# RuoyuFeng/CCEdit

Hardware: AMD Instinct MI355X
Metric: UNet denoising steps/s (TV2V 17x512x768, bf16, CFG-doubled batch) (higher is better)
Workload: dtype bf16; 1 GPU; TV2V depth-midas, 17x512x768, one network evaluation = ControlNet2D + pseudo-3D UNet on B=2 (cfg 7.5 uncond+cond) x T=17 frames, latent 64x96, 77x768 text context; 77.68 TFLOP/step; a 30-step DPMPP2SAncestral clip = 59 such steps + VAE decode; parallelism=single GPU, hint_stem=recomputed every step

## Files before the change

ccedit_amd/csrc/common.h:

```cpp
#pragma once
#include <hip/hip_runtime.h>
#include <stdint.h>

#include "../../include/ccedit_hip.h"

typedef __bf16 bf16;
typedef __attribute__((ext_vector_type(8))) __bf16 bf16x8;
typedef __attribute__((ext_vector_type(4))) __bf16 bf16x4;
typedef __attribute__((ext_vector_type(2))) __bf16 bf16x2;
typedef __attribute__((ext_vector_type(16))) float f32x16;
typedef __attribute__((ext_vector_type(4))) float f32x4;
typedef __attribute__((ext_vector_type(2))) float f32x2;
typedef __attribute__((ext_vector_type(4))) short s16x4;
typedef __attribute__((ext_vector_type(4))) uint32_t u32x4;
typedef __attribute__((ext_vector_type(2))) uint32_t u32x2;

#define GLOBAL_AS __attribute__((address_space(1)))
#define LDS_AS __attribute__((address_space(3)))

__device__ __forceinline__ void glds16(const void* gsrc, void* lds_wave_base) {
    __builtin_amdgcn_global_load_lds((const GLOBAL_AS void*)gsrc, (LDS_AS void*)lds_wave_base, 16, 0, 0);
}

__device__ __forceinline__ float bf2f(bf16 v) { return (float)v; }
__device__ __forceinline__ bf16 f2bf(float v) { return (bf16)v; }

__device__ __forceinline__ float silu_f(float v) { return v * __builtin_amdgcn_rcpf(1.0f + __expf(-v)); }
#ifdef CCEDIT_GELU_AS71_28
__device__ __forceinline__ float gelu_erf_f(float v) {
    const float x = fabsf(v) * 0.70710678118654752440f;
    float p = fmaf(x, 0.0000430638f, 0.0002765672f);
    p = fmaf(x, p, 0.0001520143f);
    p = fmaf(x, p, 0.0092705272f);
    p = fmaf(x, p, 0.0422820123f);
    p = fmaf(x, p, 0.0705230784f);
    p = fmaf(x, p, 1.0f);
    p = p * p;
    p = p * p;
    p = p * p;
    p = p * p;
    const float e = 1.0f - __builtin_amdgcn_rcpf(p);
    return 0.5f * v + 0.5f * fabsf(v) * e;
}
#else
__device__ __forceinline__ float gelu_erf_f(float v) {
    const float vc = __builtin_amdgcn_fmed3f(v, -9.0f, 9.0f);
    const float t = vc * vc;
    float p = fmaf(t, 0.00101426306f, -0.106775724f);
    p = fmaf(t, p, -2.30112134f);
    const float e = __builtin_amdgcn_exp2f(p * vc);
    return v * __builtin_amdgcn_rcpf(1.0f + e);
}
#endif

__device__ __forceinline__ float wave_sum(float v) {
#pragma unroll
    for (int o = 32; o > 0; o >>= 1) v += __shfl_xor(v, o, 64);
    return v;
}

struct CcPolicy {
    int conv_halo = 1;
    int g8 = 1;
    int g8_conv = 1;
    int g8_temporal = 1;
    int g8_split = -1;
    int g8_mfma16 = 1;
    int lin320 = 1;
    int lin320s = 1;
    int lin640 = 1;
    int temp320 = 1;
    int attn_short = 1;
    int attn_text = 1;
    int attn_spatial = 1;
    int attn_pv16 = 1;
    int attn_opt = 1;
    int gn_flat = 1;
    int gn_apply_flat = 1;
    int f32_split = 1;
};
const CcPolicy& cc_policy();

void cc_set_error(const char* fmt, ...);
void cc_note_kernel(const char* fmt, ...);

#define CC_CHECK_ARG(cond, ...)          \
    do {                                 \
        if (!(cond)) {                   \
            cc_set_error(__VA_ARGS__);   \
            return CCEDIT_EINVAL;        \
        }                                \
    } while (0)

#define CC_UNSUPPORTED(cond, ...)        \
    do {                                 \
        if (cond) {                      \
            cc_set_error(__VA_ARGS__);   \
            return CCEDIT_EUNSUPPORTED;  \
        }                                \
    } while (0)

static inline int cc_max_dynamic_lds(const void* fn, int bytes, unsigned long long* done, const char* what) {
    int dev = 0;
    hipError_t e = hipGetDevice(&dev);
    if (e == hipSuccess && dev < 64 && ((*done >> dev) & 1ull)) return CCEDIT_OK;
    if (e == hipSuccess) e = hipFuncSetAttribute(fn, hipFuncAttributeMaxDynamicSharedMemorySize, bytes);
    if (e != hipSuccess) {
        cc_set_error("hipFuncSetAttribute(%s): %s", what, hipGetErrorString(e));
        return (int)e;
    }
    if (dev < 64) *done |= 1ull << dev;
    return CCEDIT_OK;
}

template <class... Arms>
// ... 120 lines not shown
```

ccedit_amd/csrc/convhalo.hip:

```cpp
#include "common.h"
#include "gemm_epilogue.h"
#include <stdlib.h>
#include <type_traits>

namespace {

__device__ __attribute__((aligned(64))) char g_zero_page_h[64];

#ifdef CONV_PROBE
constexpr int kProbeWgs = 8192, kProbeStamps = 8;
__device__ unsigned long long g_conv_probe[kProbeWgs * kProbeStamps];
#define CONV_STAMP(i)                                                                                                     \
    do {                                                                                                                  \
        if (threadIdx.x == 0 && blockIdx.x < kProbeWgs) g_conv_probe[blockIdx.x * kProbeStamps + (i)] = __builtin_amdgcn_s_memrealtime(); \
    } while (0)
#else
#define CONV_STAMP(i) \
    do {              \
    } while (0)
#endif

template <int N>
__device__ __forceinline__ void wait_vmcnt_h() {
    asm volatile("s_waitcnt vmcnt(%0)" ::"n"(N) : "memory");
// ... 126 lines not shown
            __builtin_amdgcn_sched_barrier(0);
#pragma unroll
            for (int i = 0; i < TI; ++i)
                if (i == 0 || !narrow) {
#pragma unroll
                    for (int j = 0; j < TJ; ++j)
                        acc[i][j] = __builtin_amdgcn_mfma_f32_32x32x16_bf16(af[ks & 1][i], bfr[ks & 1][j], acc[i][j], 0, 0, 0);
                }
            __builtin_amdgcn_sched_barrier(0);
        }
    };

    CONV_STAMP(0);
    stageW(0, 0);
    stageH(0, 0);
    wait_vmcnt_h<0>();
    __syncthreads();
    CONV_STAMP(1);
    int kt = 0;
    for (int c = 0; c < nc; ++c) {
        for (int t = 0; t < 9; ++t, ++kt) {
            if (kt + 1 < nk) stageW(kt + 1, (kt + 1) & 1);
            const bool pre = (t == 0) && (c + 1 < nc);
            if (pre) stageH(c + 1, (c + 1) & 1);
            compute(kt & 1, c & 1, t);
            if (pre) wait_vmcnt_h<kHaloIssues - 1>(); else wait_vmcnt_h<0>();
            __syncthreads();
        }
    }

    CONV_STAMP(2);
    const int64_t row_base = ((int64_t)frame * d.Hout + y0) * d.Wout + x0;
    gemm_epilogue<WM, WN, TI, TJ, LDS_MAIN>(
        d, acc, smem, ch0,
        [&](int px) -> int64_t {
            const int tx = px & (TW - 1);
            return x0 + tx < d.Wout ? row_base + (int64_t)(px >> tw_log2) * d.Wout + tx : -1;
        },
        (int64_t)frame, narrow);
    CONV_STAMP(3);
#ifdef CONV_PROBE
    if (threadIdx.x == 0 && blockIdx.x < kProbeWgs) {
        unsigned hw_id;
        asm volatile("s_getreg_b32 %0, hwreg(HW_REG_HW_ID)" : "=s"(hw_id));
        unsigned xcc;
        asm volatile("s_getreg_b32 %0, hwreg(HW_REG_XCC_ID)" : "=s"(xcc));
        g_conv_probe[blockIdx.x * kProbeStamps + 4] = ((unsigned long long)xcc << 32) | hw_id;
        g_conv_probe[blockIdx.x * kProbeStamps + 5] = (unsigned long long)ch0;
    }
#endif
}


constexpr int kHaloBytes4 = 192 * 128;

template <int WM, int WN, int TI, int TJ>
__global__ __launch_bounds__(WM* WN * 64) void conv_halo4_kernel(const CcGemmDesc d, int tw_log2_flags) {
    const int tw_log2 = tw_log2_flags & 0xFF;
    constexpr int NT = WM * WN * 64;
    constexpr int BMC = WM * TI * 32, BNP = WN * TJ * 32;
    static_assert(NT == 256 && BNP == 128 && BMC == 128 && TI == 2, "tile geometry");
    constexpr int NS = 4;
    constexpr int W_SUB = BMC * 64;
    constexpr int LDS_MAIN = NS * W_SUB + 2 * kHaloBytes4;
    extern __shared__ __attribute__((aligned(16))) char smem[];
    char* const sW = smem;
    char* const sH = smem + NS * W_SUB;

    const int tid = threadIdx.x;
    const int lane = tid & 63;
    const int wave = __builtin_amdgcn_readfirstlane(tid >> 6);
    const int wm = wave / WN, wn = wave % WN;
    const int TW = 1 << tw_log2, TH = BNP >> tw_log2, HW_ = TW + 2;
    const int tiles_x = (d.Wout + TW - 1) >> tw_log2, tiles_y = d.Hout / TH;
    const int tpf = tiles_x * tiles_y;

    const int ct_n = (d.N + BMC - 1) / BMC;
    const int64_t pt_n = (int64_t)(d.M / (d.Hout * d.Wout)) * tpf;
    const int64_t pt_per_xcd = (pt_n + 7) / 8;
    const int64_t bid = blockIdx.x;
    const int xcd = (int)(bid & 7);
    const int64_t local = bid >> 3;
    const int Q = d.cgroup > 0 ? d.cgroup : ct_n;
    const int64_t gsz = pt_per_xcd * Q;
    const int cg = (int)(local / gsz);
    const int64_t rr = local - cg * gsz;
    const int qn = min(Q, ct_n - cg * Q);
    const int64_t pl = rr / qn;
    const int64_t pt = xcd * pt_per_xcd + pl;
    if (pt >= pt_n) return;
    const int ch0 = (cg * Q + (int)(rr - pl * qn)) * BMC;
    const int frame = (int)(pt / tpf);
    const int tr = (int)(pt - (int64_t)frame * tpf);
    const int y0 = (tr / tiles_x) * TH, x0 = (tr % tiles_x) << tw_log2;

    const bf16* __restrict__ Ap = (const bf16*)d.A;
    const bf16* __restrict__ Wp = (const bf16*)d.W;
    const bf16* zp = (const bf16*)g_zero_page_h;
    const int nc = d.Cin >> 6, nsub = nc * 18;
    const bool narrow = ((tw_log2_flags >> 8) & 1) && (d.N - ch0 <= WM * 32);

    const int f_hy = (tw_log2 == 3) ? 1 : 0;
    const int p = tid & 7, rsub = tid >> 3;
    int64_t hoff[kHaloIssues];
#pragma unroll
    for (int i = 0; i < kHaloIssues; ++i) {
        const int hrow = i * 32 + rsub;
        const int hy = hrow / HW_, hx = hrow - hy * HW_;
        const int iy = y0 + hy - 1, ix = x0 + hx - 1;
        const bool v = hrow < kHaloRows && (unsigned)iy < (unsigned)d.Hin && (unsigned)ix < (unsigned)d.Win;
        const int gsrc = p ^ (((hx >> 1) + ((hy & 1) << 2) * f_hy) & 7);
        hoff[i] = v ? (((int64_t)frame * d.Hin + iy) * d.Win + ix) * d.lda + gsrc * 8 : -1;
    }
    const int p4 = tid & 3, r4 = tid >> 2;
    const int gsrc_w = p4 ^ ((r4 >> 2) & 3);
    const bf16* const wsrc = Wp + (size_t)(ch0 + r4) * d.Kpad + gsrc_w * 8;
    const size_t wsrc64 = (size_t)64 * d.Kpad;

    auto stageH = [&](int c, int buf) {
#pragma unroll
        for (int i = 0; i < kHaloIssues; ++i) {
            const bf16* src = hoff[i] >= 0 ? Ap + hoff[i] + c * 64 : zp;
            glds16(src, sH + buf * kHaloBytes4 + i * (32 * 128) + wave * 1024);
        }
    };

    const int l31 = lane & 31, hi = lane >> 5;
    const int sw_w = (l31 >> 2) & 3;
    int hb[TJ], pty[TJ], ptx[TJ];
#pragma unroll
    for (int j = 0; j < TJ; ++j) {
        const int px = (wn * TJ + j) * 32 + l31;
        pty[j] = px >> tw_log2;
        ptx[j] = px & (TW - 1);
        hb[j] = pty[j] * HW_ + ptx[j];
    }

    f32x16 acc[TI][TJ];
#pragma unroll
    for (int i = 0; i < TI; ++i)
#pragma unroll
        for (int j = 0; j < TJ; ++j)
#pragma unroll
            for (int r = 0; r < 16; ++r) acc[i][j][r] = 0.f;

    CONV_STAMP(0);
    auto kloop = [&](auto NARROWC) {
        constexpr bool NARROW = decltype(NARROWC)::value;
        constexpr int WI = NARROW ? 1 : 2;
        constexpr int NTI = NARROW ? 1 : TI;
        const char* const fa = sW + ((NARROW ? wm * 32 : wm * TI * 32) + l31) * 64;
        auto stageW = [&](int sidx) {
            const bf16* src = wsrc + sidx * 32;
            char* dst = sW + (sidx & (NS - 1)) * W_SUB + wave * 1024;
#pragma unroll
            for (int i = 0; i < WI; ++i) glds16(src + i * wsrc64, dst + i * 4096);
        };
        auto wait_for = [&](int w_tiles, bool halo) {
            if (halo) {
                if (w_tiles >= 2) wait_vmcnt_h<2 * WI + kHaloIssues>();
                else if (w_tiles == 1) wait_vmcnt_h<WI + kHaloIssues>();
                else wait_vmcnt_h<kHaloIssues>();
            } else {
                if (w_tiles >= 2) wait_vmcnt_h<2 * WI>();
                else if (w_tiles == 1) wait_vmcnt_h<WI>();
                else wait_vmcnt_h<0>();
            }
        };
        auto phase = [&](int sidx, int hbuf, int half, const int (&hr)[TJ], const int (&hsw)[TJ]) {
            const char* pa = fa + (sidx & (NS - 1)) * W_SUB;
            const char* ph = sH + hbuf * kHaloBytes4;
            bf16x8 af[2][NTI], bfr[2][TJ];
#pragma unroll
            for (int k2 = 0; k2 < 2; ++k2) {
#pragma unroll
                for (int i = 0; i < NTI; ++i) af[k2][i] = *(const bf16x8*)(pa + i * 32 * 64 + (((k2 * 2 + hi) ^ sw_w) << 4));
#pragma unroll
                for (int j = 0; j < TJ; ++j) bfr[k2][j] = *(const bf16x8*)(ph + hr[j] * 128 + ((((half * 2 + k2) * 2 + hi) ^ hsw[j]) << 4));
            }
            __builtin_amdgcn_sched_barrier(0);
#pragma unroll
            for (int k2 = 0; k2 < 2; ++k2)
#pragma unroll
                for (int i = 0; i < NTI; ++i)
#pragma unroll
                    for (int j = 0; j < TJ; ++j)
                        acc[i][j] = __builtin_amdgcn_mfma_f32_32x32x16_bf16(af[k2][i], bfr[k2][j], acc[i][j], 0, 0, 0);
            __builtin_amdgcn_sched_barrier(0);
        };

        stageW(0);
        stageH(0, 0);
        stageW(1);
        stageW(2);
        wait_vmcnt_h<2 * WI>();
        __syncthreads();
        CONV_STAMP(1);
        int sidx = 0;
        for (int c = 0; c < nc; ++c) {
            const bool more_chunks = c + 1 < nc;
            for (int t = 0; t < 9; ++t) {
                const int dy = t / 3, dx = t - dy * 3;
                const int shift = dy * HW_ + dx;
                int hr[TJ], hsw[TJ];
#pragma unroll
                for (int j = 0; j < TJ; ++j) {
                    hr[j] = hb[j] + shift;
                    hsw[j] = (((ptx[j] + dx) >> 1) + (((pty[j] + dy) & 1) << 2) * f_hy) & 7;
                }
#pragma unroll
                for (int half = 0; half < 2; ++half, ++sidx) {
                    if (sidx + 3 < nsub) stageW(sidx + 3);
                    const bool first = (t == 0 && half == 0);
                    if (first && more_chunks) stageH(c + 1, (c + 1) & 1);
                    phase(sidx, c & 1, half, hr, hsw);
                    const int left = nsub - 2 - sidx;
                    wait_for(left < 0 ? 0 : left, more_chunks && t == 0 || (more_chunks && t == 1 && half == 0));
                    __syncthreads();
                }
            }
        }
    };
    if (narrow) kloop(std::true_type{});
    else kloop(std::false_type{});

    CONV_STAMP(2);
    const int64_t row_base = ((int64_t)frame * d.Hout + y0) * d.Wout + x0;
    gemm_epilogue<WM, WN, TI, TJ, LDS_MAIN>(
        d, acc, smem, ch0,
        [&](int px) -> int64_t {
            const int tx = px & (TW - 1);
            return x0 + tx < d.Wout ? row_base + (int64_t)(px >> tw_log2) * d.Wout + tx : -1;
        },
        (int64_t)frame, narrow);
    CONV_STAMP(3);
#ifdef CONV_PROBE
    if (threadIdx.x == 0 && blockIdx.x < kProbeWgs) {
        g_conv_probe[blockIdx.x * kProbeStamps + 4] = 0;
        g_conv_probe[blockIdx.x * kProbeStamps + 5] = (unsigned long long)ch0;
    }
#endif
}

}

#ifdef CONV_PROBE
extern "C" int ccedit_conv_probe_read(unsigned long long* dst, int n) {
    return (int)hipMemcpyFromSymbol(dst, HIP_SYMBOL(g_conv_probe), sizeof(unsigned long long) * (size_t)n, 0, hipMemcpyDeviceToHost);
}
#endif

bool cc_conv_halo_applicable(const CcGemmDesc& d) {
    if (!(d.mode == CCEDIT_GEMM_CONV2D && d.taps == 9 && d.ksize == 3 && d.stride == 1 && d.pad == 1 && !d.upsample &&
          !d.A2 && d.korder == 1 && d.Cin % 64 == 0 && d.Cin1 == d.Cin && d.Hout == d.Hin && d.Wout == d.Win && d.N >= 64 &&
          d.act != CCEDIT_ACT_GEGLU))
        return false;
    if (d.M % ((int64_t)d.Hout * d.Wout) != 0) return false;
    if (d.gn_stats && d.gn_rows != d.Hout * d.Wout) return false;
    return d.Hout % 8 == 0 || (d.Wout % 8 == 0 && d.Hout % 16 == 0);
}

int cc_conv_halo_launch(const CcGemmDesc& d, hipStream_t s) {
    constexpr int WM = 2, WN = 2, TI = 2, TJ = 2;
    constexpr int BMC = WM * TI * 32, BNP = WN * TJ * 32;
    constexpr int lds = epi_lds_total(BMC, BNP, TJ, 2 * BMC * 128 + 2 * kHaloBytes);
    static unsigned long long attr_done = 0;
    if (int rc = cc_max_dynamic_lds((const void*)conv_halo_kernel<WM, WN, TI, TJ>, lds, &attr_done, "conv_halo")) return rc;
    const int pad16 = (d.Hout % 8 == 0) ? (d.Wout + 15) / 16 * 16 : 1 << 30;
    const int pad8 = (d.Hout % 16 == 0) ? (d.Wout + 7) / 8 * 8 : 1 << 30;
    const int tw_log2 = pad16 <= pad8 ? 4 : 3;
    const int TWh = 1 << tw_log2, THh = BNP >> tw_log2;
    const int64_t frames = d.M / ((int64_t)d.Hout * d.Wout);
    const int64_t pt_n = frames * ((d.Wout + TWh - 1) / TWh) * (d.Hout / THh), ct_n = (d.N + BMC - 1) / BMC;
    const int64_t nblk = 8 * ((pt_n + 7) / 8) * ct_n;
    if (nblk > 2147483647LL) {
        cc_set_error("ccedit_gemm: grid too large");
        return CCEDIT_EUNSUPPORTED;
    }
    CcGemmDesc dd = d;
    dd.cgroup = 0;
    if (ct_n > 3) {
        const int q = 3;
        const int ng = (int)((ct_n + q - 1) / q);
        dd.cgroup = (int)((ct_n + ng - 1) / ng);
    }
    if (cc_policy().conv_halo != 2) {
        constexpr int lds4 = epi_lds_total(BMC, BNP, TJ, 4 * BMC * 64 + 2 * kHaloBytes4);
        static unsigned long long attr_done4 = 0;
        if (int rc = cc_max_dynamic_lds((const void*)conv_halo4_kernel<WM, WN, TI, TJ>, lds4, &attr_done4, "conv_halo4")) return rc;
        cc_note_kernel("conv_halo_kernel, four-slot weight ring");
        hipLaunchKernelGGL((conv_halo4_kernel<WM, WN, TI, TJ>), dim3((unsigned)nblk), dim3(WM * WN * 64), lds4, s, dd, tw_log2 | (1 << 8));
        return cc_launch_status("conv_halo4_kernel");
    }
    cc_note_kernel("conv_halo_kernel, two-slot weight ring");
    hipLaunchKernelGGL((conv_halo_kernel<WM, WN, TI, TJ>), dim3((unsigned)nblk), dim3(WM * WN * 64), lds, s, dd,
                       tw_log2 | (1 << 8));
    return cc_launch_status("conv_halo_kernel");
}
```

ccedit_amd/csrc/core.cpp:

```cpp
#include <stdarg.h>
#include <stdio.h>
#include <string.h>

#include "common.h"

static thread_local char g_err[512] = "";

void cc_set_error(const char* fmt, ...) {
    va_list ap;
    va_start(ap, fmt);
    vsnprintf(g_err, sizeof(g_err), fmt, ap);
    va_end(ap);
}

static thread_local char g_kernel[96] = "";

void cc_note_kernel(const char* fmt, ...) {
    va_list ap;
    va_start(ap, fmt);
    vsnprintf(g_kernel, sizeof(g_kernel), fmt, ap);
    va_end(ap);
}

extern "C" const char* ccedit_last_kernel(void) { return g_kernel; }

extern "C" int ccedit_abi_version(void) { return CCEDIT_ABI_VERSION; }

extern "C" const char* ccedit_last_error(void) { return g_err; }

extern "C" int ccedit_device_info(char* name, int name_len) {
    int dev = 0;
    hipError_t e = hipGetDevice(&dev);
    if (e != hipSuccess) {
        cc_set_error("hipGetDevice: %s", hipGetErrorString(e));
        return -(int)e;
    }
    hipDeviceProp_t prop;
    e = hipGetDeviceProperties(&prop, dev);
    if (e != hipSuccess) {
        cc_set_error("hipGetDeviceProperties: %s", hipGetErrorString(e));
        return -(int)e;
    }
    if (name && name_len > 0) {
        strncpy(name, prop.gcnArchName, (size_t)name_len - 1);
        name[name_len - 1] = 0;
    }
    return prop.multiProcessorCount;
}

static CcPolicy g_policy;
const CcPolicy& cc_policy() { return g_policy; }

namespace {
struct PolicyEntry {
    const char* name;
    int CcPolicy::*field;
};
const PolicyEntry kPolicy[] = {
    {"conv_halo", &CcPolicy::conv_halo},     {"g8", &CcPolicy::g8},           {"g8_conv", &CcPolicy::g8_conv},
    {"g8_temporal", &CcPolicy::g8_temporal}, {"g8_split", &CcPolicy::g8_split}, {"g8_mfma16", &CcPolicy::g8_mfma16}, {"lin320", &CcPolicy::lin320},
    {"lin320s", &CcPolicy::lin320s},         {"lin640", &CcPolicy::lin640},   {"temp320", &CcPolicy::temp320},
    {"attn_short", &CcPolicy::attn_short},   {"attn_text", &CcPolicy::attn_text}, {"attn_spatial", &CcPolicy::attn_spatial},
    {"attn_pv16", &CcPolicy::attn_pv16},     {"attn_opt", &CcPolicy::attn_opt},       {"gn_flat", &CcPolicy::gn_flat}, {"gn_apply_flat", &CcPolicy::gn_apply_flat},
    {"f32_split", &CcPolicy::f32_split},
};
}

extern "C" int ccedit_policy_set(const char* name, int32_t value) {
    CC_CHECK_ARG(name != nullptr, "ccedit_policy_set: null name");
    for (const PolicyEntry& e : kPolicy)
        if (!strcmp(e.name, name)) {
            g_policy.*(e.field) = value;
            return CCEDIT_OK;
        }
    cc_set_error("ccedit_policy_set: unknown switch '%s'", name);
    return CCEDIT_EINVAL;
}

extern "C" int ccedit_policy_get(const char* name, int32_t* value) {
    CC_CHECK_ARG(name != nullptr && value != nullptr, "ccedit_policy_get: null argument");
    for (const PolicyEntry& e : kPolicy)
        if (!strcmp(e.name, name)) {
            *value = g_policy.*(e.field);
            return CCEDIT_OK;
        }
    cc_set_error("ccedit_policy_get: unknown switch '%s'", name);
    return CCEDIT_EINVAL;
}

extern "C" const char* ccedit_policy_names(void) {
    static char buf[512] = "";
    if (!buf[0]) {
        size_t n = 0;
        for (const PolicyEntry& e : kPolicy) n += (size_t)snprintf(buf + n, sizeof(buf) - n, "%s%s", n ? "," : "", e.name);
    }
    return buf;
}

static const int64_t kPixelMax = (int64_t)1 << 31;

extern "C" int ccedit_resize_u8_pil(const void* src, void* dst, void* tmp, const int32_t* ytab, int32_t yk, const int32_t* xtab, int32_t xk,
                                    int32_t N, int32_t Hs, int32_t Ws, int32_t H, int32_t W, int32_t out_f32, void* stream) {
    CC_CHECK_ARG(src && dst && ytab, "ccedit_resize_u8_pil: null pointer (src, dst and ytab are required)");
    CC_CHECK_ARG(N > 0 && Hs > 0 && Ws > 0 && H > 0 && W > 0, "ccedit_resize_u8_pil: sizes must be positive (N=%d, %dx%d -> %dx%d)", N, Hs, Ws, H, W);
    CC_CHECK_ARG(yk >= 1 && yk <= 4096 && (!xtab || (xk >= 1 && xk <= 4096)), "ccedit_resize_u8_pil: tap counts yk=%d xk=%d (1 ... 4096)", yk, xk);
    CC_CHECK_ARG(xtab || Ws == W, "ccedit_resize_u8_pil: xtab may only be null when the width does not change (%d -> %d)", Ws, W);
    CC_CHECK_ARG(!xtab || tmp, "ccedit_resize_u8_pil: the horizontal pass needs tmp (N x Hs x W x 3 bytes)");
    CC_CHECK_ARG((int64_t)N * Hs * (Ws > W ? Ws : W) * 3 < kPixelMax && (int64_t)N * H * W * 3 < kPixelMax,
                 "ccedit_resize_u8_pil: more than 2^31 bytes in one call (N=%d, %dx%d -> %dx%d)", N, Hs, Ws, H, W);
    return cc_pixel_resize_u8((const uint8_t*)src, dst, (uint8_t*)tmp, ytab, yk, xtab, xk, N, Hs, Ws, H, W, out_f32, (hipStream_t)stream);
}

// ... 620 lines not shown
```

ccedit_amd/csrc/gemm.hip:

```cpp
#include "common.h"
#include "gemm_epilogue.h"
#include <math.h>
#include <stdlib.h>

bool cc_conv_halo_applicable(const CcGemmDesc& d);
int cc_conv_halo_launch(const CcGemmDesc& d, hipStream_t s);
bool cc_lin320_applicable(const CcGemmDesc& d);
int cc_lin320_launch(const CcGemmDesc& d, hipStream_t s);
bool cc_lin640_applicable(const CcGemmDesc& d);
bool cc_temp320_applicable(const CcGemmDesc& d);
int cc_temp320_launch(const CcGemmDesc& d, hipStream_t s);
int cc_lin640_launch(const CcGemmDesc& d, hipStream_t s);
bool cc_small_conv_applicable(const CcGemmDesc& d);
int cc_small_conv_launch(const CcGemmDesc& d, hipStream_t s);
bool cc_g8_applicable(const CcGemmDesc& d, int shape);
int cc_g8_launch(const CcGemmDesc& d, hipStream_t s, int shape);
int cc_g8_split(const CcGemmDesc& d, int n_cu);
int64_t cc_g8_workspace_bytes(const CcGemmDesc& d, int n_cu);

namespace {

__device__ __attribute__((aligned(64))) char g_zero_page[64];


enum { M_LINEAR = 0, M_CONV = 1, M_TEMPORAL = 2, M_CONV_UP = 3 };

template <int N>
__device__ __forceinline__ void wait_vmcnt() {
    asm volatile("s_waitcnt vmcnt(%0)" ::"n"(N) : "memory");
}

template <int WM, int WN, int TI, int TJ, int STAGES, int BKE, int MODE, bool HALO3 = false>
__global__ __launch_bounds__(WM* WN * 64) void tap_gemm_kernel(const CcGemmDesc d) {
    static_assert(BKE == 64 || BKE == 32, "K tile");
    constexpr int kRowBytes = BKE * 2;
    constexpr int GPR = BKE / 8;
    constexpr int KSTEPS = BKE / 16;
    constexpr int NT = WM * WN * 64;
    constexpr int RPI = NT / GPR;
    constexpr int BMC = WM * TI * 32;
    constexpr int BNP = WN * TJ * 32;
    constexpr int A_ISSUES = BMC / RPI;
    constexpr int B_ISSUES = BNP / RPI;
    constexpr int LPS = A_ISSUES + B_ISSUES;
    constexpr int A_BYTES = BMC * kRowBytes;
    constexpr int B_BYTES = BNP * kRowBytes;
    static_assert(RPI % 32 == 0 && BMC % RPI == 0 && BNP % RPI == 0, "tile / thread-count mismatch");
    extern __shared__ __attribute__((aligned(16))) char smem[];
    char* const sA = smem;
    char* const sB = smem + STAGES * A_BYTES;

    const int tid = threadIdx.x;
    const int lane = tid & 63;
    const int wave = __builtin_amdgcn_readfirstlane(tid >> 6);
    const int wm = wave / WN, wn = wave % WN;
    const int ct_n = (d.N + BMC - 1) / BMC;
    const int64_t pt_n = (d.M + BNP - 1) / BNP;
    const int64_t pt_per_xcd = (pt_n + 7) / 8;
    const int64_t bid = blockIdx.x;
// ... 300 lines not shown
    CcGemmDesc d = *desc;
    CC_CHECK_ARG(d.A && d.W && d.out, "ccedit_gemm: null A/W/out");
    CC_CHECK_ARG(d.M > 0 && d.N > 0 && d.Cin > 0 && d.taps > 0, "ccedit_gemm: bad sizes M=%lld N=%d Cin=%d taps=%d",
                 (long long)d.M, d.N, d.Cin, d.taps);
    CC_UNSUPPORTED(d.Cin % 8 != 0, "ccedit_gemm: Cin=%d must be a multiple of 8", d.Cin);
    CC_UNSUPPORTED(d.N % 4 != 0, "ccedit_gemm: N=%d must be a multiple of 4", d.N);
    CC_UNSUPPORTED(d.Kpad % 64 != 0 || d.Kpad < d.taps * d.Cin, "ccedit_gemm: Kpad=%d invalid for taps*Cin=%d", d.Kpad,
                   d.taps * d.Cin);
    CC_UNSUPPORTED(d.lda % 8 != 0 || d.ldc % 4 != 0, "ccedit_gemm: lda=%d / ldc=%d alignment", d.lda, d.ldc);
    CC_UNSUPPORTED(d.M >= (1LL << 31), "ccedit_gemm: M too large");
    if (d.A2 == nullptr) d.Cin1 = d.Cin;
    CC_UNSUPPORTED(d.korder && (d.Cin % 64 != 0 || d.Cin1 % 64 != 0 || d.Kpad != d.taps * d.Cin),
                   "ccedit_gemm: korder=1 needs Cin (and the concat split) to be multiples of 64");
    CC_UNSUPPORTED(d.N > 4 && ((!d.out_f32 && d.ldc % 8 != 0) || (d.res1 && d.ldr1 % 8 != 0) || (d.res2 && d.ldr2 % 8 != 0)),
                   "ccedit_gemm: N > 4 needs ldc / residual strides that are multiples of 8");
    CC_UNSUPPORTED(d.A2 && (d.Cin1 % 8 != 0 || d.lda2 % 8 != 0 || d.Cin1 <= 0 || d.Cin1 >= d.Cin),
                   "ccedit_gemm: bad concat split Cin1=%d lda2=%d", d.Cin1, d.lda2);
    if (d.mode == CCEDIT_GEMM_CONV2D) {
        CC_CHECK_ARG(d.ksize * d.ksize == d.taps && d.Hin > 0 && d.Win > 0 && d.Hout > 0 && d.Wout > 0 && d.stride > 0,
                     "ccedit_gemm: bad conv2d geometry");
        CC_CHECK_ARG(d.M % ((int64_t)d.Hout * d.Wout) == 0, "ccedit_gemm: M not a whole number of frames");
        CC_CHECK_ARG(d.subpix >= 0 && d.subpix <= 4, "ccedit_gemm: subpix must be 0..4");
        CC_CHECK_ARG(d.vpad >= 0 && d.vpad <= 2, "ccedit_gemm: vpad must be 0, 1 or 2");
        CC_CHECK_ARG(d.vpad == 2 || (!d.halo_top && !d.halo_bot), "ccedit_gemm: halo_top / halo_bot go with vpad 2");
        CC_UNSUPPORTED(d.vpad && (d.upsample || d.tile > 3 || d.A2), "ccedit_gemm: vpad runs on the generic tap-gather block shapes only, without the fused upsample / a second source");
        CC_UNSUPPORTED(d.subpix && (d.ksize != 2 || d.stride != 1 || d.upsample || d.Hin != d.Hout + (d.vpad == 1 ? 2 : 0) || d.Win != d.Wout || d.gn_stats || d.A2 ||
                                    4 * d.M >= (1LL << 31)),
                       "ccedit_gemm: subpix needs ksize 2, stride 1, a same-size low-resolution frame, no gn_stats / second source");
    } else if (d.subpix || d.vpad || d.halo_top || d.halo_bot) {
        CC_CHECK_ARG(false, "ccedit_gemm: subpix / vpad / halo rows are CONV2D modes");
    } else if (d.mode == CCEDIT_GEMM_TEMPORAL) {
        CC_CHECK_ARG(d.T > 0 && d.HW > 0 && d.M % ((int64_t)d.T * d.HW) == 0, "ccedit_gemm: bad temporal geometry");
        CC_CHECK_ARG(d.taps % 2 == 1, "ccedit_gemm: temporal taps must be odd");
        if (d.Tsrc == 0) {
            d.Tsrc = d.T;
            d.tsrc_off = 0;
            d.t0 = 0;
            d.Tglob = d.T;
        }
        CC_CHECK_ARG(d.Tsrc >= d.T + d.tsrc_off && d.tsrc_off >= 0 && d.t0 >= 0 && d.t0 + d.T <= d.Tglob,
                     "ccedit_gemm: bad frame-shard geometry");
        CC_UNSUPPORTED((int64_t)(d.M / ((int64_t)d.T * d.HW)) * d.Tsrc * d.HW >= (1LL << 31), "ccedit_gemm: source too large");
    } else {
        CC_CHECK_ARG(d.mode == CCEDIT_GEMM_LINEAR && d.taps == 1, "ccedit_gemm: bad mode/taps");
    }
    if (d.act == CCEDIT_ACT_GEGLU) {
        CC_UNSUPPORTED(d.N % 16 != 0 || d.res1 || d.res2 || d.group_bias || d.out_f32,
                       "ccedit_gemm: GEGLU epilogue needs N%%16==0 and no residual/group bias/f32 out");
    }
    if (d.group_bias) CC_CHECK_ARG(d.group_rows > 0 && (d.ldgb == 0 || d.ldgb >= d.N), "ccedit_gemm: group_bias without group_rows / ldgb < N");
    if (d.gn_stats && !(d.tile >= 11 && d.tile <= 13)) {
        CC_CHECK_ARG(d.gn_rows > 0 && d.gn_rows % 128 == 0 && d.M % d.gn_rows == 0,
                     "ccedit_gemm: gn_stats needs gn_rows %% 128 == 0 dividing M (gn_rows=%d)", d.gn_rows);
        CC_CHECK_ARG(d.gn_rows % 256 == 0 || d.tile <= 1 || d.tile == 8 || d.tile == 14,
                     "ccedit_gemm: gn_rows=%d is not a multiple of 256: only the 128-pixel block shape (tile 1) applies", d.gn_rows);
        CC_UNSUPPORTED(d.tile == 6, "ccedit_gemm: gn_stats is not available with the 320-channel block shape (tile 6)");
        CC_UNSUPPORTED(d.N % 32 != 0 || d.N < 256 || d.out_f32 || d.act == CCEDIT_ACT_GEGLU,
                       "ccedit_gemm: gn_stats needs N%%32==0, N>=256, bf16 output, no GEGLU (N=%d)", d.N);
    }
    hipStream_t s = (hipStream_t)stream;
    if (d.ln_eps != 0.f) {
        CC_UNSUPPORTED(!(d.tile == 0 || d.tile == 9) || !cc_lin320_applicable(d),
                       "ccedit_gemm: ln_eps needs the register-resident K = 320 kernel (block shape 0 / 9, plain Linear with K = 320 "
                       "and N %% 320 == 0, no activation / residual): not applicable to this descriptor");
        return cc_lin320_launch(d, s);
    }
    const CcPolicy& pol = cc_policy();
    if ((d.tile == 0 && pol.temp320 && d.M >= 100000) || d.tile == 14) {
        if (cc_temp320_applicable(d)) return cc_temp320_launch(d, s);
        CC_UNSUPPORTED(d.tile == 14, "ccedit_gemm: tile 14 (streaming Conv1d k3, 320 input channels) does not apply to this descriptor");
    }
    if ((d.tile == 0 && pol.lin640 && d.M >= 16384 && (d.N >= 1024 || (!d.ln_stats && !d.ln_sums))) || d.tile == 10) {
        if (cc_lin640_applicable(d)) return cc_lin640_launch(d, s);
        CC_UNSUPPORTED(d.tile == 10, "ccedit_gemm: tile 10 (register-resident weights, K = 640) does not apply to this descriptor");
    }
    if (d.ln_stats || d.ln_sums || d.ln_colsum) {
        const int shape = (d.tile >= 11 && d.tile <= 13) ? d.tile - 11 : 0;
        CC_UNSUPPORTED((!d.ln_stats && !d.ln_sums) || !d.ln_colsum || !(d.tile == 0 || (d.tile >= 11 && d.tile <= 13)) || !cc_g8_applicable(d, shape),
                       "ccedit_gemm: ln_stats needs ln_colsum and the persistent eight-phase kernel (block shape 0 / 11-13: plain Linear with "
                       "Cin %% 64 == 0, N %% 16 == 0, no residual / row bias / gn_stats): not applicable to this descriptor");
        return cc_g8_launch(d, s, shape);
    }
    if (d.row_sums) {
        const int shape = (d.tile >= 11 && d.tile <= 13) ? d.tile - 11 : 0;
        CC_UNSUPPORTED(!(d.tile == 0 || (d.tile >= 11 && d.tile <= 13)) || !cc_g8_applicable(d, shape),
                       "ccedit_gemm: row_sums needs the persistent eight-phase kernel (block shape 0 / 11-13: Linear with Cin %% 64 == 0, "
                       "N %% 16 == 0, no activation): not applicable to this descriptor");
        return cc_g8_launch(d, s, shape);
    }
    if (d.tile == 0 && !d.vpad && cc_small_conv_applicable(d)) return cc_small_conv_launch(d, s);
    if (d.tile == 0 && pol.g8_conv && pol.g8 && !d.vpad && d.mode == CCEDIT_GEMM_CONV2D && d.N >= 1024 && d.M >= 12000 && cc_g8_applicable(d, 1))
        return cc_g8_launch(d, s, 1);
    if (d.tile == 0 && pol.g8 && (!d.subpix || pol.g8_conv) && !d.vpad && d.workspace && cc_g8_split(d, 0) > 1 && d.workspace_bytes >= cc_g8_workspace_bytes(d, 0))
        return cc_g8_launch(d, s, 1);
    if (d.tile == 0 && pol.g8_conv && pol.g8 && d.subpix && d.M >= 12000 && d.N >= 640 && cc_g8_applicable(d, 0)) return cc_g8_launch(d, s, 0);
    if ((d.tile == 0 && pol.conv_halo && !d.vpad) || d.tile == 8) {
        if (!d.vpad && cc_conv_halo_applicable(d)) return cc_conv_halo_launch(d, s);
        CC_UNSUPPORTED(d.tile == 8, "ccedit_gemm: tile 8 (LDS-halo 3x3 conv) does not apply to this descriptor");
    }
    if ((d.tile == 0 && pol.lin320 && d.M >= 32768) || d.tile == 9) {
        if (cc_lin320_applicable(d)) return cc_lin320_launch(d, s);
        CC_UNSUPPORTED(d.tile == 9, "ccedit_gemm: tile 9 (register-resident weights, K = 320) does not apply to this descriptor");
    }
    if (d.tile >= 11 && d.tile <= 13) {
        CC_UNSUPPORTED(!cc_g8_applicable(d, d.tile - 11), "ccedit_gemm: tile 11-13 (persistent eight-phase GEMM) does not apply to this descriptor");
        return cc_g8_launch(d, s, d.tile - 11);
    }
    if (d.tile == 0 && pol.g8 && !d.subpix && d.M >= 4096 && d.Kpad >= 640 && d.N >= 640 && cc_g8_applicable(d, 0)) {
        if (d.mode == CCEDIT_GEMM_LINEAR || (d.mode == CCEDIT_GEMM_TEMPORAL && pol.g8_temporal && d.M >= 12000)) return cc_g8_launch(d, s, 0);
    }
    CC_UNSUPPORTED(d.tile == 6 && d.N % 320 != 0, "ccedit_gemm: tile 6 (320-channel block shape) needs N %% 320 == 0 (N=%d)", d.N);
    int tile = d.tile;
    if (tile == 0) {
        const int w128 = (d.N + 127) / 128 * 128, w64 = (d.N + 63) / 64 * 64;
        if (w64 < w128) tile = (d.taps > 1 || d.Kpad <= 512) ? 2 : 1;
        else if (d.M >= 150000 && d.Kpad >= 2048) tile = 3;
        else if (d.act == CCEDIT_ACT_GEGLU && d.Kpad <= 640) tile = 2;
        else tile = 1;
        if (d.N % 320 == 0 && !d.gn_stats && d.M >= 8192 &&
            ((d.mode == CCEDIT_GEMM_LINEAR && d.Kpad >= 1280) || (d.mode == CCEDIT_GEMM_TEMPORAL && d.Kpad >= 3840)))
            tile = 6;
        if (d.mode == CCEDIT_GEMM_LINEAR && d.N % 256 == 0 && d.N <= 2560 && d.act != CCEDIT_ACT_GEGLU && !d.gn_stats &&
            d.Kpad >= 1280 && d.M >= 12000 && d.M <= 16384)
            tile = 4;
        if (d.gn_stats && d.gn_rows % 256 != 0) tile = 1;
    }
    const int mode = d.mode == CCEDIT_GEMM_CONV2D ? (d.upsample ? M_CONV_UP : M_CONV)
                                                  : (d.mode == CCEDIT_GEMM_TEMPORAL ? M_TEMPORAL : M_LINEAR);
    switch (mode) {
        case M_CONV: return launch_tile<M_CONV>(d, tile, s);
        case M_CONV_UP: return launch_tile<M_CONV_UP>(d, tile, s);
        case M_TEMPORAL: return launch_tile<M_TEMPORAL>(d, tile, s);
        default: return launch_tile<M_LINEAR>(d, tile, s);
    }
}
```

ccedit_amd/policy.py:

```python
from __future__ import annotations

import os
from typing import Dict

TABLE = {
    "graph": (1, "py", "0: eager launches instead of HIP-graph replay of a network evaluation"),
    "overlap_controlnet": (1, "py", "0: ControlNet on the main stream instead of a side stream"),
    "split_cfg": (0, "py", "1: the two CFG halves as B = 1 passes on two streams (round-2 execution)"),
    "hint_dedup": (1, "py", "0: hint stem evaluated for both CFG halves"),
    "text_kv_batched": (1, "py", "0: one text K/V projection launch per transformer block"),
    "share_cfg_prefix": (1, "py", "0: identical CFG halves evaluated in full (no shared prefix up to the first text attention)"),
    "fuse_gn_stats": (1, "py", "0: two-pass GroupNorm everywhere (no statistics from the producers' epilogues)"),
    "ff320": (1, "py", "0: LayerNorm + two GEMMs instead of the fused dim-320 feed-forward"),
    "ln320": (1, "py", "0: separate LayerNorm pass in front of the K = 320 projections"),
    "lnf": (1, "py", "0: LayerNorm passes in front of the 640 / 1280-channel projections"),
    "ln_sums": (1, "py", "0: LayerNorm statistics by ccedit_row_stats instead of the producer's epilogue"),
    "subpix": (1, "py", "0: upsample + 3x3 conv through the nine-tap gather instead of four parity convs"),
    "conv1x1_linear": (1, "py", "0: 1 x 1 convs through the convolution mode instead of the Linear dispatch"),
    "attn_q_log2": (1, "py", "0: softmax scale applied inside the attention kernels instead of folded into to_q"),
    "fuse_halo_stats": (1, "py", "0 (rows sharded): GroupNorm statistics all-reduced on their own instead of riding on the 3x3 conv's halo exchange"),
    "wfrag": (1, "py", "0: the register-resident-weight kernels (K = 320 / 640 Linears, 320-channel Conv1d k3) preload their weights from the row-major matrix instead of its fragment-ordered copy"),
    "block_tail": (1, "py", "0: to_out / proj_out of the dim-320 transformer tails as their own launches, not inside ff320"),
    "vae_fp32": (2, "py", "the KL-VAE's precision.  2 (default): the engine follows the yaml's disable_first_stage_autocast, the flag's meaning in "
                          "the reference (diffusion.py:151-156; the shipped yamls set it => fp32 on v_mfma_f32_32x32x2_f32, ccedit_amd/vae_f32.py); "
                          "1: always fp32, also for a first stage built outside an engine; 0: always the bf16-storage kernels"),
    "conv_halo": (1, "lib", "0: 3x3 stride-1 convs on the tap-gather kernel; 2: the LDS-halo kernel with the two-slot weight ring of rounds 2-5"),
    "g8": (1, "lib", "0: long Linears on the tap_gemm block shapes"),
    "g8_conv": (1, "lib", "0: 3x3 convs onto >= 1024 channels not on the persistent kernel"),
    "g8_temporal": (1, "lib", "0: Conv1d k3 at >= 640 channels not on the persistent kernel"),
    "g8_split": (-1, "lib", "split-K at the 8x12 level: -1 auto, 0 off, n fixed"),
    "g8_mfma16": (1, "lib", "0: the persistent kernel's K loop on 32x32x16 MFMAs instead of 16x16x32 (2: same as 1, the value tests set)"),
    "lin320": (1, "lib", "0: K = 320 Linears on tap_gemm"),
    "lin320s": (1, "lib", "0: the K-split lin320 kernel instead of the streaming one"),
    "lin640": (1, "lib", "0: K = 640 Linears on the persistent kernel"),
    "temp320": (1, "lib", "0: 320-channel Conv1d k3 on tap_gemm"),
    "attn_short": (1, "lib", "0: temporal attention through the general flash kernel"),
    "attn_text": (1, "lib", "0: text cross-attention through the general flash kernel"),
    "attn_spatial": (1, "lib", "0: the 6144-key (d = 40) and 1536-key (d = 80) self-attention through the general flash kernel; 2: only d = 40 on the specialised kernel"),
    "attn_pv16": (1, "lib", "0: PV product of the spatial attention in 32x32x16 tiles"),
    "attn_opt": (1, "lib", "0: softmax reference of the spatial attention tracked on every key tile (no optimistic first-tile reference)"),
    "gn_flat": (1, "lib", "0: temporal GroupNorm through the per-pixel kernels at the two large levels"),
    "gn_apply_flat": (1, "lib", "0: spatial GroupNorm apply with a wave per pixel row instead of a granule column per thread"),
    "f32_split": (1, "lib", "0: the fp32 first stage's contractions on v_mfma_f32_32x32x2_f32 instead of six exact bf16 x bf16 products per fp32 product "
                            "(three-way operand split, the dropped terms below fp32's own accumulation rounding) on the bf16 matrix pipe; 2: the split form on the eight-wave kernel only"),
}

_values: Dict[str, int] = {}


def _parse(what: str, text: str, legacy_switch: bool = False) -> int:
    t = text.strip()
    try:
        return int(t)
    except ValueError:
        if legacy_switch:
            return 0 if t.lower() in ("0", "off", "false", "no") else 1
        raise ValueError(f"{what}: '{text}' is not an integer") from None


def _load():
    vals = {k: v[0] for k, v in TABLE.items()}
    for name in TABLE:
        legacy = {"g8_split": "CCEDIT_G8_SPLIT"}.get(name, "CCEDIT_" + name.upper())
        if legacy in os.environ:
            vals[name] = _parse(legacy, os.environ[legacy], legacy_switch=True)
    spec = os.environ.get("CCEDIT_POLICY", "")
    for item in filter(None, (x.strip() for x in spec.split(","))):
        if "=" not in item:
            raise ValueError(f"CCEDIT_POLICY: '{item}' is not name=value")
        k, v = item.split("=", 1)
        if k.strip() not in TABLE:
            raise ValueError(f"CCEDIT_POLICY: unknown switch '{k.strip()}' (known: {', '.join(TABLE)})")
        vals[k.strip()] = _parse(f"CCEDIT_POLICY: {k.strip()}", v)
    return vals


def get(name: str) -> int:
    if not _values:
        _values.update(_load())
# ... 25 lines not shown
```

Baseline: 10.79 UNet steps/s.

## Add 256-pixel (16x16) tile variant of LDS-halo 3x3 conv kernel

Adds a wide variant of the four-slot LDS-halo conv kernel that covers a 16x16 pixel tile per workgroup, with a single halo buffer, halo offsets recomputed per stage, and frame-local 32-bit addressing. The aim is more weight reuse per staged weight tile and fewer halo bytes per output pixel. A heuristic picks it when its workgroup-round count beats the 128-pixel version by a margin at a two-workgroups-per-CU occupancy target. The single halo buffer adds an extra wait and barrier per input-channel chunk, and the dispatch changes to contiguous per-XCD ranges, both of which can reduce overlap.

```diff
diff --git a/ccedit_amd/csrc/common.h b/ccedit_amd/csrc/common.h
--- a/ccedit_amd/csrc/common.h
+++ b/ccedit_amd/csrc/common.h
@@ -61,6 +61,7 @@
 
 struct CcPolicy {
     int conv_halo = 1;
+    int conv_wide = 1;
     int g8 = 1;
     int g8_conv = 1;
     int g8_temporal = 1;
diff --git a/ccedit_amd/csrc/convhalo.hip b/ccedit_amd/csrc/convhalo.hip
--- a/ccedit_amd/csrc/convhalo.hip
+++ b/ccedit_amd/csrc/convhalo.hip
@@ -202,17 +202,24 @@
 }
 
 
-constexpr int kHaloBytes4 = 192 * 128;
+constexpr int halo4_rows(int bnp) { return (bnp / 16 + 2) * 18; }
+constexpr int halo4_issues(int bnp) { return (halo4_rows(bnp) + 31) / 32; }
+constexpr int halo4_bytes(int bnp) { return halo4_issues(bnp) * 32 * 128; }
+constexpr int halo4_bufs(int bnp) { return bnp == 128 ? 2 : 1; }
+constexpr int halo4_lds_main(int bmc, int bnp) { return 4 * bmc * 64 + halo4_bufs(bnp) * halo4_bytes(bnp); }
 
 template <int WM, int WN, int TI, int TJ>
-__global__ __launch_bounds__(WM* WN * 64) void conv_halo4_kernel(const CcGemmDesc d, int tw_log2_flags) {
-    const int tw_log2 = tw_log2_flags & 0xFF;
+__global__ __launch_bounds__(WM* WN * 64, TJ == 4 ? 2 : 1) void conv_halo4_kernel(const CcGemmDesc d, int tw_log2_flags) {
     constexpr int NT = WM * WN * 64;
     constexpr int BMC = WM * TI * 32, BNP = WN * TJ * 32;
-    static_assert(NT == 256 && BNP == 128 && BMC == 128 && TI == 2, "tile geometry");
+    static_assert(NT == 256 && (BNP == 128 || BNP == 256) && BMC == 128 && TI == 2, "tile geometry");
+    constexpr bool WIDE = BNP == 256;
+    const int tw_log2 = WIDE ? 4 : tw_log2_flags & 0xFF;
     constexpr int NS = 4;
     constexpr int W_SUB = BMC * 64;
-    constexpr int LDS_MAIN = NS * W_SUB + 2 * kHaloBytes4;
+    constexpr int kRows = halo4_rows(BNP), kIssues = halo4_issues(BNP), kBytes = halo4_bytes(BNP), NH = halo4_bufs(BNP);
+    constexpr int LDS_MAIN = halo4_lds_main(BMC, BNP);
+    static_assert(LDS_MAIN <= 80 * 1024, "two workgroups per CU");
     extern __shared__ __attribute__((aligned(16))) char smem[];
     char* const sW = smem;
     char* const sH = smem + NS * W_SUB;
@@ -227,17 +234,19 @@
 
     const int ct_n = (d.N + BMC - 1) / BMC;
     const int64_t pt_n = (int64_t)(d.M / (d.Hout * d.Wout)) * tpf;
-    const int64_t pt_per_xcd = (pt_n + 7) / 8;
+    const int64_t pt_per_xcd = WIDE ? pt_n : (pt_n + 7) / 8;
     const int64_t bid = blockIdx.x;
     const int xcd = (int)(bid & 7);
-    const int64_t local = bid >> 3;
+    const int64_t wg_per_xcd = (pt_n * ct_n + 7) / 8;
+    const int64_t local = WIDE ? xcd * wg_per_xcd + (bid >> 3) : bid >> 3;
+    if (WIDE && local >= pt_n * ct_n) return;
     const int Q = d.cgroup > 0 ? d.cgroup : ct_n;
     const int64_t gsz = pt_per_xcd * Q;
     const int cg = (int)(local / gsz);
     const int64_t rr = local - cg * gsz;
     const int qn = min(Q, ct_n - cg * Q);
     const int64_t pl = rr / qn;
-    const int64_t pt = xcd * pt_per_xcd + pl;
+    const int64_t pt = WIDE ? pl : xcd * pt_per_xcd + pl;
     if (pt >= pt_n) return;
     const int ch0 = (cg * Q + (int)(rr - pl * qn)) * BMC;
     const int frame = (int)(pt / tpf);
@@ -252,15 +261,19 @@
 
     const int f_hy = (tw_log2 == 3) ? 1 : 0;
     const int p = tid & 7, rsub = tid >> 3;
-    int64_t hoff[kHaloIssues];
-#pragma unroll
-    for (int i = 0; i < kHaloIssues; ++i) {
-        const int hrow = i * 32 + rsub;
+    const bf16* const Ah = WIDE ? Ap + (int64_t)frame * d.Hin * d.Win * d.lda : Ap;
+    auto halo_src = [&](int hrow) -> int64_t {
         const int hy = hrow / HW_, hx = hrow - hy * HW_;
         const int iy = y0 + hy - 1, ix = x0 + hx - 1;
-        const bool v = hrow < kHaloRows && (unsigned)iy < (unsigned)d.Hin && (unsigned)ix < (unsigned)d.Win;
+        const bool v = hrow < kRows && (unsigned)iy < (unsigned)d.Hin && (unsigned)ix < (unsigned)d.Win;
         const int gsrc = p ^ (((hx >> 1) + ((hy & 1) << 2) * f_hy) & 7);
-        hoff[i] = v ? (((int64_t)frame * d.Hin + iy) * d.Win + ix) * d.lda + gsrc * 8 : -1;
+        if constexpr (WIDE) return v ? (iy * d.Win + ix) * d.lda + gsrc * 8 : -1;
+        else return v ? (((int64_t)frame * d.Hin + iy) * d.Win + ix) * d.lda + gsrc * 8 : -1;
+    };
+    int64_t hoff[WIDE ? 1 : kIssues];
+    if constexpr (!WIDE) {
+#pragma unroll
+        for (int i = 0; i < kIssues; ++i) hoff[i] = halo_src(i * 32 + rsub);
     }
     const int p4 = tid & 3, r4 = tid >> 2;
     const int gsrc_w = p4 ^ ((r4 >> 2) & 3);
@@ -268,10 +281,13 @@
     const size_t wsrc64 = (size_t)64 * d.Kpad;
 
     auto stageH = [&](int c, int buf) {
-#pragma unroll
-        for (int i = 0; i < kHaloIssues; ++i) {
-            const bf16* src = hoff[i] >= 0 ? Ap + hoff[i] + c * 64 : zp;
-            glds16(src, sH + buf * kHaloBytes4 + i * (32 * 128) + wave * 1024);
+        int r = rsub;
+        if constexpr (WIDE) asm volatile("" : "+v"(r));
+#pragma unroll
+        for (int i = 0; i < kIssues; ++i) {
+            const int64_t off = WIDE ? halo_src(i * 32 + r) : hoff[i];
+            const bf16* src = off >= 0 ? Ah + off + c * 64 : zp;
+            glds16(src, sH + buf * kBytes + i * (32 * 128) + wave * 1024);
         }
     };
 
@@ -308,9 +324,9 @@
         };
         auto wait_for = [&](int w_tiles, bool halo) {
             if (halo) {
-                if (w_tiles >= 2) wait_vmcnt_h<2 * WI + kHaloIssues>();
-                else if (w_tiles == 1) wait_vmcnt_h<WI + kHaloIssues>();
-                else wait_vmcnt_h<kHaloIssues>();
+                if (w_tiles >= 2) wait_vmcnt_h<2 * WI + kIssues>();
+                else if (w_tiles == 1) wait_vmcnt_h<WI + kIssues>();
+                else wait_vmcnt_h<kIssues>();
             } else {
                 if (w_tiles >= 2) wait_vmcnt_h<2 * WI>();
                 else if (w_tiles == 1) wait_vmcnt_h<WI>();
@@ -319,7 +335,7 @@
         };
         auto phase = [&](int sidx, int hbuf, int half, const int (&hr)[TJ], const int (&hsw)[TJ]) {
             const char* pa = fa + (sidx & (NS - 1)) * W_SUB;
-            const char* ph = sH + hbuf * kHaloBytes4;
+            const char* ph = sH + hbuf * kBytes;
             bf16x8 af[2][NTI], bfr[2][TJ];
 #pragma unroll
             for (int k2 = 0; k2 < 2; ++k2) {
@@ -362,11 +378,19 @@
                 for (int half = 0; half < 2; ++half, ++sidx) {
                     if (sidx + 3 < nsub) stageW(sidx + 3);
                     const bool first = (t == 0 && half == 0);
-                    if (first && more_chunks) stageH(c + 1, (c + 1) & 1);
-                    phase(sidx, c & 1, half, hr, hsw);
+                    if constexpr (NH == 2) {
+                        if (first && more_chunks) stageH(c + 1, (c + 1) & 1);
+                    } else if (first && c > 0) {
+                        wait_vmcnt_h<WI>();
+                        __syncthreads();
+                    }
+                    phase(sidx, NH == 2 ? c & 1 : 0, half, hr, hsw);
                     const int left = nsub - 2 - sidx;
-                    wait_for(left < 0 ? 0 : left, more_chunks && t == 0 || (more_chunks && t == 1 && half == 0));
+                    wait_for(left < 0 ? 0 : left, NH == 2 && (more_chunks && t == 0 || (more_chunks && t == 1 && half == 0)));
                     __syncthreads();
+                    if constexpr (NH == 1) {
+                        if (t == 8 && half == 1 && more_chunks) stageH(c + 1, 0);
+                    }
                 }
             }
         }
@@ -410,7 +434,57 @@
     return d.Hout % 8 == 0 || (d.Wout % 8 == 0 && d.Hout % 16 == 0);
 }
 
-int cc_conv_halo_launch(const CcGemmDesc& d, hipStream_t s) {
+bool cc_conv_wide_applicable(const CcGemmDesc& d) {
+    return cc_conv_halo_applicable(d) && d.Hout % 16 == 0 && (int64_t)d.Hin * d.Win * d.lda < (1LL << 31);
+}
+
+bool cc_conv_wide_auto(const CcGemmDesc& d) {
+    if (d.M < 16384) return false;
+    int cus = 256;
+    {
+        int dev = 0;
+        static int cu_cache[64] = {0};
+        if (hipGetDevice(&dev) == hipSuccess && dev < 64) {
+            if (!cu_cache[dev]) {
+                int v = 0;
+                if (hipDeviceGetAttribute(&v, hipDeviceAttributeMultiprocessorCount, dev) == hipSuccess && v > 0) cu_cache[dev] = v;
+            }
+            if (cu_cache[dev]) cus = cu_cache[dev];
+        }
+    }
+    const int64_t slots = 2 * (int64_t)cus;
+    const int64_t wide = d.M / ((int64_t)d.Hout * d.Wout) * ((d.Wout + 15) / 16) * (d.Hout / 16) * ((d.N + 127) / 128);
+    const int64_t rounds_wide = (wide + slots - 1) / slots, rounds_128 = (2 * wide + slots - 1) / slots;
+    return 182 * rounds_wide < 100 * rounds_128;
+}
+
+static int conv_wide_launch(const CcGemmDesc& d, hipStream_t s) {
+    constexpr int WM = 2, WN = 2, TI = 2, TJ = 4;
+    constexpr int BMC = WM * TI * 32, BNP = WN * TJ * 32;
+    constexpr int lds = epi_lds_total(BMC, BNP, TJ, halo4_lds_main(BMC, BNP));
+    static_assert(lds <= 80 * 1024, "two workgroups per CU");
+    const int64_t frames = d.M / ((int64_t)d.Hout * d.Wout);
+    const int64_t pt_n = frames * ((d.Wout + 15) / 16) * (d.Hout / 16), ct_n = (d.N + BMC - 1) / BMC;
+    const int64_t nblk = 8 * ((pt_n * ct_n + 7) / 8);
+    if (nblk > 2147483647LL) {
+        cc_set_error("ccedit_gemm: grid too large");
+        return CCEDIT_EUNSUPPORTED;
+    }
+    CcGemmDesc dd = d;
+    dd.cgroup = 0;
+    if (ct_n > 3) {
+        const int ng = (int)((ct_n + 2) / 3);
+        dd.cgroup = (int)((ct_n + ng - 1) / ng);
+    }
+    static unsigned long long attr_done = 0;
+    if (int rc = cc_max_dynamic_lds((const void*)conv_halo4_kernel<WM, WN, TI, TJ>, lds, &attr_done, "conv_halo4 wide")) return rc;
+    cc_note_kernel("conv_halo_kernel, four-slot weight ring, 256-pixel tile");
+    hipLaunchKernelGGL((conv_halo4_kernel<WM, WN, TI, TJ>), dim3((unsigned)nblk), dim3(WM * WN * 64), lds, s, dd, 4 | (1 << 8));
+    return cc_launch_status("conv_halo4_kernel");
+}
+
+int cc_conv_halo_launch(const CcGemmDesc& d, hipStream_t s, bool wide) {
+    if (wide) return conv_wide_launch(d, s);
     constexpr int WM = 2, WN = 2, TI = 2, TJ = 2;
     constexpr int BMC = WM * TI * 32, BNP = WN * TJ * 32;
     constexpr int lds = epi_lds_total(BMC, BNP, TJ, 2 * BMC * 128 + 2 * kHaloBytes);
@@ -435,7 +509,7 @@
         dd.cgroup = (int)((ct_n + ng - 1) / ng);
     }
     if (cc_policy().conv_halo != 2) {
-        constexpr int lds4 = epi_lds_total(BMC, BNP, TJ, 4 * BMC * 64 + 2 * kHaloBytes4);
+        constexpr int lds4 = epi_lds_total(BMC, BNP, TJ, halo4_lds_main(BMC, BNP));
         static unsigned long long attr_done4 = 0;
         if (int rc = cc_max_dynamic_lds((const void*)conv_halo4_kernel<WM, WN, TI, TJ>, lds4, &attr_done4, "conv_halo4")) return rc;
         cc_note_kernel("conv_halo_kernel, four-slot weight ring");
diff --git a/ccedit_amd/csrc/core.cpp b/ccedit_amd/csrc/core.cpp
--- a/ccedit_amd/csrc/core.cpp
+++ b/ccedit_amd/csrc/core.cpp
@@ -57,7 +57,7 @@
     int CcPolicy::*field;
 };
 const PolicyEntry kPolicy[] = {
-    {"conv_halo", &CcPolicy::conv_halo},     {"g8", &CcPolicy::g8},           {"g8_conv", &CcPolicy::g8_conv},
+    {"conv_halo", &CcPolicy::conv_halo},     {"conv_wide", &CcPolicy::conv_wide},     {"g8", &CcPolicy::g8},           {"g8_conv", &CcPolicy::g8_conv},
     {"g8_temporal", &CcPolicy::g8_temporal}, {"g8_split", &CcPolicy::g8_split}, {"g8_mfma16", &CcPolicy::g8_mfma16}, {"lin320", &CcPolicy::lin320},
     {"lin320s", &CcPolicy::lin320s},         {"lin640", &CcPolicy::lin640},   {"temp320", &CcPolicy::temp320},
     {"attn_short", &CcPolicy::attn_short},   {"attn_text", &CcPolicy::attn_text}, {"attn_spatial", &CcPolicy::attn_spatial},
diff --git a/ccedit_amd/csrc/gemm.hip b/ccedit_amd/csrc/gemm.hip
--- a/ccedit_amd/csrc/gemm.hip
+++ b/ccedit_amd/csrc/gemm.hip
@@ -4,7 +4,9 @@
 #include <stdlib.h>
 
 bool cc_conv_halo_applicable(const CcGemmDesc& d);
-int cc_conv_halo_launch(const CcGemmDesc& d, hipStream_t s);
+bool cc_conv_wide_applicable(const CcGemmDesc& d);
+bool cc_conv_wide_auto(const CcGemmDesc& d);
+int cc_conv_halo_launch(const CcGemmDesc& d, hipStream_t s, bool wide);
 bool cc_lin320_applicable(const CcGemmDesc& d);
 int cc_lin320_launch(const CcGemmDesc& d, hipStream_t s);
 bool cc_lin640_applicable(const CcGemmDesc& d);
@@ -411,7 +413,7 @@
     if (d.gn_stats && !(d.tile >= 11 && d.tile <= 13)) {
         CC_CHECK_ARG(d.gn_rows > 0 && d.gn_rows % 128 == 0 && d.M % d.gn_rows == 0,
                      "ccedit_gemm: gn_stats needs gn_rows %% 128 == 0 dividing M (gn_rows=%d)", d.gn_rows);
-        CC_CHECK_ARG(d.gn_rows % 256 == 0 || d.tile <= 1 || d.tile == 8 || d.tile == 14,
+        CC_CHECK_ARG(d.gn_rows % 256 == 0 || d.tile <= 1 || d.tile == 8 || d.tile == 14 || d.tile == 15,
                      "ccedit_gemm: gn_rows=%d is not a multiple of 256: only the 128-pixel block shape (tile 1) applies", d.gn_rows);
         CC_UNSUPPORTED(d.tile == 6, "ccedit_gemm: gn_stats is not available with the 320-channel block shape (tile 6)");
         CC_UNSUPPORTED(d.N % 32 != 0 || d.N < 256 || d.out_f32 || d.act == CCEDIT_ACT_GEGLU,
@@ -453,8 +455,16 @@
     if (d.tile == 0 && pol.g8 && (!d.subpix || pol.g8_conv) && !d.vpad && d.workspace && cc_g8_split(d, 0) > 1 && d.workspace_bytes >= cc_g8_workspace_bytes(d, 0))
         return cc_g8_launch(d, s, 1);
     if (d.tile == 0 && pol.g8_conv && pol.g8 && d.subpix && d.M >= 12000 && d.N >= 640 && cc_g8_applicable(d, 0)) return cc_g8_launch(d, s, 0);
+    if (d.tile == 15) {
+        CC_UNSUPPORTED(d.vpad || !cc_conv_wide_applicable(d), "ccedit_gemm: tile 15 (LDS-halo 3x3 conv, 256-pixel tile: stride 1, Cin %% 64 == 0, "
+                       "Hout %% 16 == 0, fewer than 2^31 elements per source frame) does not apply to this descriptor");
+        return cc_conv_halo_launch(d, s, true);
+    }
     if ((d.tile == 0 && pol.conv_halo && !d.vpad) || d.tile == 8) {
-        if (!d.vpad && cc_conv_halo_applicable(d)) return cc_conv_halo_launch(d, s);
+        if (!d.vpad && cc_conv_halo_applicable(d)) {
+            const bool wide = d.tile == 0 && pol.conv_halo == 1 && pol.conv_wide && cc_conv_wide_applicable(d) && (pol.conv_wide == 2 || cc_conv_wide_auto(d));
+            return cc_conv_halo_launch(d, s, wide);
+        }
         CC_UNSUPPORTED(d.tile == 8, "ccedit_gemm: tile 8 (LDS-halo 3x3 conv) does not apply to this descriptor");
     }
     if ((d.tile == 0 && pol.lin320 && d.M >= 32768) || d.tile == 9) {
diff --git a/ccedit_amd/policy.py b/ccedit_amd/policy.py
--- a/ccedit_amd/policy.py
+++ b/ccedit_amd/policy.py
@@ -25,6 +25,7 @@
                           "the reference (diffusion.py:151-156; the shipped yamls set it => fp32 on v_mfma_f32_32x32x2_f32, ccedit_amd/vae_f32.py); "
                           "1: always fp32, also for a first stage built outside an engine; 0: always the bf16-storage kernels"),
     "conv_halo": (1, "lib", "0: 3x3 stride-1 convs on the tap-gather kernel; 2: the LDS-halo kernel with the two-slot weight ring of rounds 2-5"),
+    "conv_wide": (1, "lib", "0: the LDS-halo kernel on 128-pixel tiles everywhere; 2: on 256-pixel (16 x 16) tiles wherever they apply, not only where they measured faster"),
     "g8": (1, "lib", "0: long Linears on the tap_gemm block shapes"),
     "g8_conv": (1, "lib", "0: 3x3 convs onto >= 1024 channels not on the persistent kernel"),
     "g8_temporal": (1, "lib", "0: Conv1d k3 at >= 640 channels not on the persistent kernel"),
```

Measured after the change: 10.97 UNet steps/s (median of 6 runs). 1.02x the previous value.
